# facebookresearch/EgoT2

Measured on AMD Instinct MI355X. Metric: clips/sec fwd+bwd, 3-task TTM translator (B=256,T=15,d=128), higher is better.
Workload: dtype f32 (operands split exactly into 3 bf16 parts; 6 bf16 MFMA products per K-block, f32 accumulate); 1 GPU; configs[1]: TTM 3-task translator, 1 layer d=128 h=4 d_ff=2048, B=256/GPU T=15 S=45, synthetic N(0,1) features, random-init weights, train mode dropout=0.5 (+0.1 on PE), weighted CE (evaluated in the forward's head epilogue), fwd+bwd; global_batch=256, parallelism=dp1, impl=auto, workgroups_per_clip=1, launch=one hipGraph replay per step, deterministic=False, compute_is_module_default=True, loss=weighted CE in the forward's head epilogue (egx_ce)

## Files before the change

### egot2_amd/csrc/fused_bwd.hip

```cpp
#include <stdlib.h>
#include <string.h>
#include <type_traits>
#include "common.h"
#include "kernels.h"
#include "fused.h"
#ifndef EGX_FFN_PIPE_BWD
#define EGX_FFN_PIPE_BWD 0
#endif
#ifndef EGX_FFN_PIPE_BWD_RING
#define EGX_FFN_PIPE_BWD_RING 16
#endif

#ifdef EGX_STAMPS
namespace egx { extern __device__ unsigned long long g_bstamps[32]; }
#define LNB_STAMP(base, k) do { if ((base) >= 0 && blockIdx.x == 0 && threadIdx.x == 0) { __builtin_amdgcn_sched_barrier(0); egx::g_bstamps[(base) + (k)] = __builtin_amdgcn_s_memtime(); __builtin_amdgcn_sched_barrier(0); } } while (0)
#endif
#include "fused_dev.h"

namespace egx {

template <int CM, int HT>
__global__ __launch_bounds__(256, HT == 1 ? 2 : 1) void ffn_dw_kernel(FfnDwParams p) {
    extern __shared__ __attribute__((aligned(16))) float lds[];
    constexpr int TILE = 32 * LDX;
// ... 1195 lines not shown
        const float* tile0 = p.slabs + (size_t)(pr.first_block + item * pr.splits) * (64 * 128) + r * 128 + c;
        float4 s = make_float4(0, 0, 0, 0);
        int sp = 0;
        for (; sp + 8 <= nsp; sp += 8) {
            float4 v[8];
#pragma unroll
            for (int k = 0; k < 8; ++k) v[k] = *reinterpret_cast<const float4*>(tile0 + (size_t)(sp + k) * (64 * 128));
#pragma unroll
            for (int k = 0; k < 8; ++k) { s.x += v[k].x; s.y += v[k].y; s.z += v[k].z; s.w += v[k].w; }
        }
        for (; sp < nsp; ++sp) {
            const float4 v = *reinterpret_cast<const float4*>(tile0 + (size_t)sp * (64 * 128));
            s.x += v.x; s.y += v.y; s.z += v.z; s.w += v.w;
        }
        const int row = row0 + r, col = col0 + c;
        if (row < pr.R && col < pr.C) {
            float4* dst = reinterpret_cast<float4*>(pr.out + (size_t)row * pr.C + col);
            const float4 o = *dst;
            *dst = make_float4(o.x + s.x, o.y + s.y, o.z + s.z, o.w + s.w);
        }
        return;
    }
    reduce_slabs_block(t.red, b - t.part_blocks - t.tile_blocks);
}

int tail_reduce(const SmallDwParams* sp, const SlabReduce* red, const ReducePartialsParams* rp, uint64_t* seed_advance_ptr, const TouchList* touch, hipStream_t st) {
    TailReduceParams t;
    memset(&t, 0, sizeof(t));
    if (sp && sp->n && sp->slabs) {
        t.sp = *sp;
        int items = 0;
        for (int i = 0; i < sp->n; ++i) items += cdiv(sp->pr[i].R, 64) * cdiv(sp->pr[i].C, 128);
        t.tile_blocks = (unsigned)items * 8;
    }
    if (red && red->narr) {
        t.red = *red;
        size_t total = 0;
        for (int k = 0; k < red->narr; ++k) total += red->n[k];
        t.slab_blocks = (unsigned)((total / 4 + 255) / 256);
    }
    if (rp && rp->n) { t.rp = *rp; t.part_blocks = (unsigned)cdiv(rp->P, 16); }
    t.seed_advance = seed_advance_ptr;
    if (touch) t.touch = *touch;
    const unsigned blocks = t.tile_blocks + t.slab_blocks + t.part_blocks;
    if (!blocks) return seed_advance_ptr ? seed_advance(seed_advance_ptr, st) : 0;
    hipLaunchKernelGGL(tail_reduce_kernel, dim3(blocks), dim3(256), 0, st, t);
    EGX_LAUNCH_CHECK();
    return 0;
}

__device__ unsigned g_stolen_bwd;
long long slices_stolen_bwd(int reset) {
    unsigned v = 0;
    if (hipMemcpyFromSymbol(&v, HIP_SYMBOL(g_stolen_bwd), sizeof(v)) != hipSuccess) return -1;
    if (reset) { const unsigned z = 0; (void)hipMemcpyToSymbol(HIP_SYMBOL(g_stolen_bwd), &z, sizeof(z)); }
    return v;
}
__device__ unsigned long long g_bstamps[32];
#ifdef EGX_STAMPS
#define BSTAMP(i) do { if (blockIdx.x == 0 && threadIdx.x == 0) g_bstamps[i] = __builtin_amdgcn_s_memtime(); } while (0)
#else
#define BSTAMP(i) do { } while (0)
#endif
int debug_read_bstamps(unsigned long long* out, int n) {
    return hipMemcpyFromSymbol(out, HIP_SYMBOL(g_bstamps), sizeof(unsigned long long) * (n > 32 ? 32 : n)) == hipSuccess ? 0 : 1;
}

template <int CM, bool TILED, int DH, bool SLICED = false, bool CUT = false, bool RAGGED = false>
__global__ __launch_bounds__(256, 1) void fused_bwd_kernel(FusedBwdParams p) {
    static_assert(!(TILED && SLICED), "the tiled launches are not sliced");
    static_assert(!RAGGED || TILED, "ragged batches run the tiled launches");
    static_assert(!(CUT && (TILED || SLICED)), "the cut launches are neither tiled nor sliced");
    constexpr int HPW = FDH / DH, NHEAD = FH * HPW, NCT = DH / 16;
    constexpr int NT = 3;
    constexpr int SP = NT * 16;
    constexpr int BLK = SP * LDX;
    extern __shared__ __attribute__((aligned(16))) float lds[];
    float* Gs = lds;
    float* B1 = lds + 1 * BLK;
    float* B2 = lds + 2 * BLK;
    float* B3 = lds + 3 * BLK;
    float* B4 = lds + 4 * BLK;
    float* B5 = lds + 5 * BLK;
    float* stat = lds + 6 * BLK;
    float* PSB = stat + NHEAD * 3 * SP;

    const int tid = threadIdx.x, wave = tid >> 6;
    int lane = tid & 63, r = lane & 15, q = lane >> 4;
    int clip_ = blockIdx.x, slice_ = 0;
    if constexpr (SLICED) slice_map(p.n_slices, clip_, slice_);
    const int clip = clip_, slice = slice_;
    const int n_slices = SLICED ? p.n_slices : 1;
    int S, c_real, t0;
    size_t tok0;
    const int* rrec = nullptr;
    if constexpr (RAGGED) {
        c_real = p.rtab[(size_t)p.B_clips * RAGGED_REC + clip];
        rrec = p.rtab + (size_t)c_real * RAGGED_REC;
        t0 = (clip - rrec[RG_TILE0]) * 48;
        S = min(48, rrec[RG_S] - t0);
        tok0 = (size_t)rrec[RG_TOK0] + t0;
    } else if constexpr (TILED) {
        c_real = clip / p.tpc;
        t0 = (clip - c_real * p.tpc) * 48;
        S = min(48, p.S_clip - t0);
        tok0 = (size_t)c_real * p.S_clip + t0;
    } else {
        c_real = clip; t0 = 0; S = p.S; tok0 = (size_t)clip * S;
    }
    if (!CUT && p.zero_buf) {
        const size_t n4 = p.zero_n / 4, per = (n4 + gridDim.x - 1) / gridDim.x;
        const size_t b0 = (size_t)blockIdx.x * per, b1 = b0 + per < n4 ? b0 + per : n4;
        for (size_t k = b0 + threadIdx.x; k < b1; k += 256) reinterpret_cast<float4*>(p.zero_buf)[k] = make_float4(0, 0, 0, 0);
    }
    if constexpr (SLICED) { if (clip >= p.B || ((p.slice_drop >> slice) & 1)) return; }

    BSTAMP(12);
    float* part = p.partials + (size_t)clip * p.P;
#define EGX_PHASE()                                              \
    do {                                                         \
        int t_ = threadIdx.x;                                    \
        asm volatile("" : "+v"(t_));                             \
        lane = t_ & 63; r = lane & 15; q = lane >> 4;            \
    } while (0)

    const bool dev_seed = p.seed_ptr != nullptr;
    const uint64_t seed_dev = dev_seed ? *p.seed_ptr : 0ull;
    const uint64_t pos_key = dev_seed ? site_key(seed_dev, 0, SITE_POS) : p.pos_key;
    constexpr int BPF = SP * (FD / 4) / 256;
    static_assert(SP * (FD / 4) % 256 == 0, "a block must divide among the threads");
    auto blk_request = [&](f32x4 (&v)[BPF], const float* src) {
        int t_ = threadIdx.x;
        asm volatile("" : "+v"(t_));
        const f32x4* s4 = reinterpret_cast<const f32x4*>(src);
        const int n = S * (FD / 4);
#pragma unroll
        for (int k = 0; k < BPF; ++k) { const int i = t_ + 256 * k; v[k] = s4[i < n ? i : n - 1]; }
    };
    auto blk_store = [&](const f32x4 (&v)[BPF], float* dst, float* dst2) {
        int t_ = threadIdx.x;
        asm volatile("" : "+v"(t_));
#pragma unroll
        for (int k = 0; k < BPF; ++k) {
            const int i = t_ + 256 * k, row = i >> 5, c = (i & 31) << 2;
            if (i < S * (FD / 4)) {
                *reinterpret_cast<f32x4*>(dst + row * LDX + c) = v[k];
                if (dst2) *reinterpret_cast<f32x4*>(dst2 + row * LDX + c) = v[k];
            }
        }
    };
    f32x4 pf_a[BPF], pf_b[BPF];
    auto res_ptr = [&](int slot) -> const float* {
        return TILED ? p.saved_res + ((size_t)slot * p.Ntok + tok0) * FD : p.saved_res + ((size_t)slot * p.B + clip) * S * FD;
    };
    const int l_first = CUT ? p.cut_layer : TILED ? p.l_back : p.n_layers - 1;
    Touched tch = {{0, 0, 0, 0}};
    if constexpr (!TILED) { if (p.touch.n) tch = touch_lines<256>(p.touch, blockIdx.x, gridDim.x, tid); }
    blk_request(pf_a, CUT ? p.dy1 + tok0 * FD : l_first >= 0 ? res_ptr(2 * l_first + 1) : p.saved_pre + tok0 * FD);
    blk_request(pf_b, l_first >= 0 ? res_ptr(2 * l_first) : p.saved_pre + tok0 * FD);
    const int ps_g = tid >> 5, ps_c = (tid & 31) << 2;
    const f32x4 ln0_v = *reinterpret_cast<const f32x4*>(p.ln_w + ps_c);
    f32x4 n1_v = *reinterpret_cast<const f32x4*>(p.layer[l_first >= 0 ? l_first : 0].norm1_w + ps_c);
    static_assert((6 * BLK) % 4 == 0, "the blocks are zeroed in 16-byte pieces");
    for (int i = tid; i < 6 * BLK / 4; i += 256) reinterpret_cast<f32x4*>(lds)[i] = f32x4{0, 0, 0, 0};
    if (ps_g == 0) *reinterpret_cast<f32x4*>(PSB + ps_c) = ln0_v;
    __syncthreads();
    if constexpr (TILED) {
        if (p.l_front >= 0) {
// ... 617 lines not shown
                for (int j = 0; j < 32; ++j) dy[j] += t[j];
                load32(B4 + row * LDX + c0, t);
#pragma unroll
                for (int j = 0; j < 32; ++j) dy[j] += t[j];
                load32(B1 + row * LDX + c0, t);
#pragma unroll
                for (int j = 0; j < 32; ++j) dy[j] += t[j];
                load32(B5 + row * LDX + c0, x);
            },
            [&](int row, int c0, float (&dy)[32], float (&dx)[32], float (&dyx)[32]) {
                store32(Gs + row * LDX + c0, dy);
                store32(B1 + row * LDX + c0, dx);
                store32(B4 + row * LDX + c0, dyx);
                if (w.res_thresh) {
                    uint32_t orow = (uint32_t)(tok0 + row);
#pragma unroll
                    for (int j = 0; j < 32; ++j) dx[j] *= drop_scale(k_res1, orow, (uint32_t)(c0 + j), w.res_thresh, w.drop_inv);
                }
                store32(B2 + row * LDX + c0, dx);
            },
            [&] {
                if constexpr (!TILED) {
                    int t_ = threadIdx.x;
                    asm volatile("" : "+v"(t_));
#pragma unroll
                    for (int k = 0; k < QKV_PF; ++k) qv[k] = qsrc[t_ + 256 * k];
                }
            }, 16);
        BSTAMP(21);
        __syncthreads();
        store_block(w.g1_out + tok0 * FD, B2, S);
        BSTAMP(5);
        PackW<CM, 2, 4> wo_pf;
        pack_issue(wo_pf, w.out_proj_wtp, wave * 2, 4, 0);
        if (tid < 128) {
            pl[384 + tid] = colsum_lds(B4, 0, S, tid);
            pl[640 + tid] = colsum_lds(B2, 0, S, tid);
        } else {
            pl[512 + (tid - 128)] = colsum_lds(Gs, 0, S, tid - 128);
        }
        EGX_PHASE();
        __syncthreads();
        {
            f32x4 acc[2][NT];
#pragma unroll
            for (int i = 0; i < 2; ++i)
#pragma unroll
                for (int t = 0; t < NT; ++t) acc[i][t] = f32x4{0, 0, 0, 0};
            gemm_packed<CM, 2, NT, 4>(acc, wo_pf, B2, r, q);
#pragma unroll
            for (int i = 0; i < 2; ++i)
#pragma unroll
                for (int t = 0; t < NT; ++t)
                    *reinterpret_cast<float4*>(B3 + (t * 16 + r) * LDX + (wave * 2 + i) * 16 + 4 * q) =
                        make_float4(acc[i][t][0], acc[i][t][1], acc[i][t][2], acc[i][t][3]);
        }
        BSTAMP(6);
        if constexpr (TILED) {
            __syncthreads();
            store_block(p.datt + tok0 * FD, B3, S);
            store_block(p.dres + tok0 * FD, B1, S);
            return;
        }
        {
            int t_ = threadIdx.x;
            asm volatile("" : "+v"(t_));
#pragma unroll
            for (int k = 0; k < QKV_PF; ++k) {
                const int i = t_ + 256 * k, row = i / 96, c = (i - row * 96) * 4;
                float* dst = c < FD ? B4 + c : (c < 2 * FD ? B5 + (c - FD) : Gs + (c - 2 * FD));
                *reinterpret_cast<f32x4*>(dst + row * LDX) = qv[k];
            }
        }
        __syncthreads();
        BSTAMP(7);
        EGX_PHASE();
        BSTAMP(8);
        EGX_PHASE();
#pragma unroll
        for (int hl = 0; hl < HPW; ++hl) {
            const int h = wave * HPW + hl;
            const int hc = h * DH;
            const float scale = DH == 32 ? 0.17677669529663687f : 0.25f;
            float* st_m = stat + (h * 3 + 0) * SP;
            float* st_i = stat + (h * 3 + 1) * SP;
            float* st_d = stat + (h * 3 + 2) * SP;
            Frag<CM> fq[NT], fk[NT], fv[NT], fdo[NT];
#pragma unroll
            for (int t = 0; t < NT; ++t) {
                fq[t] = load_head_frag<CM, DH>(B4 + (t * 16 + r) * LDX + hc, q);
                fk[t] = load_head_frag<CM, DH>(B5 + (t * 16 + r) * LDX + hc, q);
                fv[t] = load_head_frag<CM, DH>(Gs + (t * 16 + r) * LDX + hc, q);
                fdo[t] = load_head_frag<CM, DH>(B3 + (t * 16 + r) * LDX + hc, q);
            }
            auto ldq = [&](int t) -> const Frag<CM>& { return fq[t]; };
            auto ldk = [&](int t) -> const Frag<CM>& { return fk[t]; };
            auto ldv = [&](int t) -> const Frag<CM>& { return fv[t]; };
            auto ldo = [&](int t) -> const Frag<CM>& { return fdo[t]; };
            f32x4 pt[NT][NT], dpt[NT][NT];
#pragma unroll
            for (int qt = 0; qt < NT; ++qt) {
                Frag<CM> bq = ldq(qt), bdo = ldo(qt);
#pragma unroll
                for (int kt = 0; kt < NT; ++kt) {
                    pt[kt][qt] = f32x4{0, 0, 0, 0};
                    dpt[kt][qt] = f32x4{0, 0, 0, 0};
                    mma<CM>(pt[kt][qt], ldk(kt), bq);
                    mma<CM>(dpt[kt][qt], ldv(kt), bdo);
                }
            }
            auto keep = [&](int query, int key) -> float {
                return w.attn_thresh ? drop_scale(k_attn, (uint32_t)((clip * NHEAD + h) * 64 + query), (uint32_t)key, w.attn_thresh, w.drop_inv) : 1.f;
            };
#pragma unroll
            for (int qt = 0; qt < NT; ++qt) {
                float m = -INFINITY;
#pragma unroll
                for (int kt = 0; kt < NT; ++kt)
#pragma unroll
                    for (int e = 0; e < 4; ++e) {
                        int key = kt * 16 + 4 * q + e;
                        float sv = (key < S) ? pt[kt][qt][e] * scale : -INFINITY;
                        pt[kt][qt][e] = sv;
                        m = fmaxf(m, sv);
                    }
                m = fmaxf(m, __shfl_xor(m, 16, 64));
                m = fmaxf(m, __shfl_xor(m, 32, 64));
                float sum = 0.f;
#pragma unroll
                for (int kt = 0; kt < NT; ++kt)
#pragma unroll
                    for (int e = 0; e < 4; ++e) { float pv = __expf(pt[kt][qt][e] - m); pt[kt][qt][e] = pv; sum += pv; }
                sum += __shfl_xor(sum, 16, 64);
                sum += __shfl_xor(sum, 32, 64);
                float inv = 1.f / sum;
                int query = qt * 16 + r;
                float dl = 0.f;
                float ksv[NT][4];
#pragma unroll
                for (int kt = 0; kt < NT; ++kt)
#pragma unroll
                    for (int e = 0; e < 4; ++e) {
                        float pv = pt[kt][qt][e] * inv;
                        float ks = keep(query, kt * 16 + 4 * q + e);
                        ksv[kt][e] = ks;
                        pt[kt][qt][e] = pv;
                        dpt[kt][qt][e] *= ks;
                        dl += pv * dpt[kt][qt][e];
                    }
                dl += __shfl_xor(dl, 16, 64);
                dl += __shfl_xor(dl, 32, 64);
                if (q == 0) { st_m[query] = m; st_i[query] = inv; st_d[query] = dl; }
#pragma unroll
                for (int kt = 0; kt < NT; ++kt)
#pragma unroll
                    for (int e = 0; e < 4; ++e) {
                        float pv = pt[kt][qt][e];
                        dpt[kt][qt][e] = pv * (dpt[kt][qt][e] - dl) * scale;
                        pt[kt][qt][e] = pv * ksv[kt][e];
                    }
            }
            f32x4 oq[NCT][NT], dqa[NCT][NT];
#pragma unroll
            for (int ct = 0; ct < NCT; ++ct)
#pragma unroll
                for (int qt = 0; qt < NT; ++qt) { oq[ct][qt] = f32x4{0, 0, 0, 0}; dqa[ct][qt] = f32x4{0, 0, 0, 0}; }
#pragma unroll
            for (int kb = 0; kb < 2; ++kb) {
                Frag<CM> av[NCT], ak[NCT];
#pragma unroll
                for (int ct = 0; ct < NCT; ++ct) {
                    av[ct] = gather_frag<CM>(Gs, hc + ct * 16 + r, kb * 32, q, SP - 1);
                    ak[ct] = gather_frag<CM>(B5, hc + ct * 16 + r, kb * 32, q, SP - 1);
                }
#pragma unroll
                for (int qt = 0; qt < NT; ++qt) {
                    f32x4 z = f32x4{0, 0, 0, 0};
                    Frag<CM> bp = chain_frag<CM>(pt[2 * kb][qt], (2 * kb + 1 < NT) ? pt[(2 * kb + 1 < NT) ? 2 * kb + 1 : 0][qt] : z);
                    Frag<CM> bs = chain_frag<CM>(dpt[2 * kb][qt], (2 * kb + 1 < NT) ? dpt[(2 * kb + 1 < NT) ? 2 * kb + 1 : 0][qt] : z);
#pragma unroll
                    for (int ct = 0; ct < NCT; ++ct) {
                        mma<CM>(oq[ct][qt], av[ct], bp);
                        mma<CM>(dqa[ct][qt], ak[ct], bs);
                    }
                }
            }
#pragma unroll
            for (int ct = 0; ct < NCT; ++ct)
#pragma unroll
                for (int qt = 0; qt < NT; ++qt) {
                    int tok = qt * 16 + r;
                    if (tok < S)
                        *reinterpret_cast<float4*>(w.attn_o_out + (tok0 + tok) * FD + hc + ct * 16 + 4 * q) =
                            make_float4(oq[ct][qt][0], oq[ct][qt][1], oq[ct][qt][2], oq[ct][qt][3]);
                }
            f32x4 pn[NT][NT], dsn[NT][NT];
#pragma unroll
            for (int qt = 0; qt < NT; ++qt) {
                float4 m4 = *reinterpret_cast<const float4*>(st_m + qt * 16 + 4 * q);
                float4 i4 = *reinterpret_cast<const float4*>(st_i + qt * 16 + 4 * q);
                float4 d4 = *reinterpret_cast<const float4*>(st_d + qt * 16 + 4 * q);
                float mq[4] = {m4.x, m4.y, m4.z, m4.w}, iq[4] = {i4.x, i4.y, i4.z, i4.w}, dq4[4] = {d4.x, d4.y, d4.z, d4.w};
#pragma unroll
                for (int kt = 0; kt < NT; ++kt) {
                    f32x4 sN = f32x4{0, 0, 0, 0}, dN = f32x4{0, 0, 0, 0};
                    mma<CM>(sN, ldq(qt), ldk(kt));
                    mma<CM>(dN, ldo(qt), ldv(kt));
                    int key = kt * 16 + r;
                    uint32_t m4[4] = {0xFu, 0xFu, 0xFu, 0xFu};
                    if (w.attn_thresh) tile_keep_rows(k_attn, (uint32_t)((clip * NHEAD + h) * 64 + qt * 16), (uint32_t)(kt * 4), r, q, w.attn_thresh, m4);
                    const float kinv = w.attn_thresh ? w.drop_inv : 1.f;
#pragma unroll
                    for (int e = 0; e < 4; ++e) {
                        int query = qt * 16 + 4 * q + e;
                        bool ok = (key < S) && (query < S);
                        float pv = ok ? __expf(sN[e] * scale - mq[e]) * iq[e] : 0.f;
                        float ks = ((m4[e] >> (r & 3)) & 1u) ? kinv : 0.f;
                        pn[qt][kt][e] = pv * ks;
                        dsn[qt][kt][e] = pv * (ks * dN[e] - dq4[e]) * scale;
                    }
                }
            }
            f32x4 dva[NCT][NT], dka[NCT][NT];
#pragma unroll
            for (int ct = 0; ct < NCT; ++ct)
#pragma unroll
                for (int kt = 0; kt < NT; ++kt) { dva[ct][kt] = f32x4{0, 0, 0, 0}; dka[ct][kt] = f32x4{0, 0, 0, 0}; }
#pragma unroll
            for (int kb = 0; kb < 2; ++kb) {
                Frag<CM> ad[NCT], aq[NCT];
#pragma unroll
                for (int ct = 0; ct < NCT; ++ct) {
                    ad[ct] = gather_frag<CM>(B3, hc + ct * 16 + r, kb * 32, q, SP - 1);
                    aq[ct] = gather_frag<CM>(B4, hc + ct * 16 + r, kb * 32, q, SP - 1);
                }
#pragma unroll
                for (int kt = 0; kt < NT; ++kt) {
                    f32x4 z = f32x4{0, 0, 0, 0};
                    Frag<CM> bp = chain_frag<CM>(pn[2 * kb][kt], (2 * kb + 1 < NT) ? pn[(2 * kb + 1 < NT) ? 2 * kb + 1 : 0][kt] : z);
                    Frag<CM> bs = chain_frag<CM>(dsn[2 * kb][kt], (2 * kb + 1 < NT) ? dsn[(2 * kb + 1 < NT) ? 2 * kb + 1 : 0][kt] : z);
#pragma unroll
                    for (int ct = 0; ct < NCT; ++ct) {
                        mma<CM>(dva[ct][kt], ad[ct], bp);
                        mma<CM>(dka[ct][kt], aq[ct], bs);
                    }
                }
            }
#pragma unroll
            for (int ct = 0; ct < NCT; ++ct)
#pragma unroll
                for (int t = 0; t < NT; ++t) {
                    int tok = t * 16 + r;
                    int c = hc + ct * 16 + 4 * q;
                    bool tv = tok < S;
                    float4 vq = tv ? make_float4(dqa[ct][t][0], dqa[ct][t][1], dqa[ct][t][2], dqa[ct][t][3]) : make_float4(0, 0, 0, 0);
                    float4 vk = tv ? make_float4(dka[ct][t][0], dka[ct][t][1], dka[ct][t][2], dka[ct][t][3]) : make_float4(0, 0, 0, 0);
                    float4 vv = tv ? make_float4(dva[ct][t][0], dva[ct][t][1], dva[ct][t][2], dva[ct][t][3]) : make_float4(0, 0, 0, 0);
                    *reinterpret_cast<float4*>(B4 + tok * LDX + c) = vq;
                    *reinterpret_cast<float4*>(B5 + tok * LDX + c) = vk;
                    *reinterpret_cast<float4*>(Gs + tok * LDX + c) = vv;
                    if (tv) {
                        float* o = w.dqkv_out + (tok0 + tok) * (3 * FD) + c;
                        *reinterpret_cast<float4*>(o) = vq;
                        *reinterpret_cast<float4*>(o + FD) = vk;
                        *reinterpret_cast<float4*>(o + 2 * FD) = vv;
                    }
                }
        }
        __syncthreads();
        BSTAMP(9);
        PackW<CM, 2, 4> wi_pf;
        pack_issue(wi_pf, w.in_proj_wtp, wave * 2, 12, 0);
        blk_request(pf_a, l > 0 ? res_ptr(2 * (l - 1) + 1) : p.saved_pre + tok0 * FD);
        blk_request(pf_b, l > 0 ? res_ptr(2 * (l - 1)) : p.saved_pre + tok0 * FD);
        if (tid < 128) {
            pl[768 + tid] = colsum_lds(B4, 0, S, tid);
            pl[768 + 256 + tid] = colsum_lds(Gs, 0, S, tid);
        } else {
            pl[768 + 128 + (tid - 128)] = colsum_lds(B5, 0, S, tid - 128);
        }
        EGX_PHASE();
        {
            f32x4 acc[2][NT];
#pragma unroll
            for (int i = 0; i < 2; ++i)
#pragma unroll
                for (int t = 0; t < NT; ++t) acc[i][t] = f32x4{0, 0, 0, 0};
            PackW<CM, 2, 4> wi2, wi3;
            pack_issue(wi2, w.in_proj_wtp, wave * 2, 12, 4);
            gemm_packed<CM, 2, NT, 4>(acc, wi_pf, B4, r, q);
            pack_issue(wi3, w.in_proj_wtp, wave * 2, 12, 8);
            gemm_packed<CM, 2, NT, 4>(acc, wi2, B5, r, q);
            gemm_packed<CM, 2, NT, 4>(acc, wi3, Gs, r, q);
#pragma unroll
            for (int i = 0; i < 2; ++i)
#pragma unroll
                for (int t = 0; t < NT; ++t) {
                    int tok = t * 16 + r;
                    int c = (wave * 2 + i) * 16 + 4 * q;
                    float4 rs = *reinterpret_cast<const float4*>(B1 + tok * LDX + c);
                    float4 o = make_float4(acc[i][t][0] + rs.x, acc[i][t][1] + rs.y, acc[i][t][2] + rs.z, acc[i][t][3] + rs.w);
                    if (tok >= S) o = make_float4(0, 0, 0, 0);
                    *reinterpret_cast<float4*>(B2 + tok * LDX + c) = o;
                }
        }
        __syncthreads();
        { float* t = Gs; Gs = B2; B2 = t; }
        if constexpr (CUT) {
            if (l > 0) {
                store_block(p.dxin + tok0 * FD, Gs, S);
                return;
            }
        }
    }

        BSTAMP(10);
    {
        float* pg = part + p.n_layers * FUSED_P_LAYER;
        blk_store(pf_a, B1, nullptr);
        __syncthreads();
        ln_bwd_rows_lds(S, PSB, p.eps,
            [&](int row, int c0, float (&dy)[32], float (&x)[32]) {
                load32(Gs + row * LDX + c0, dy);
                if (p.pos_thresh) {
                    uint32_t orow = (uint32_t)(tok0 + row);
#pragma unroll
                    for (int j = 0; j < 32; ++j) dy[j] *= drop_scale(pos_key, orow, (uint32_t)(c0 + j), p.pos_thresh, p.pos_inv);
                }
                load32(B1 + row * LDX + c0, x);
            },
            [&](int row, int c0, float (&dy)[32], float (&dx)[32], float (&dyx)[32]) {
                store32(Gs + row * LDX + c0, dy);
                store32(B3 + row * LDX + c0, dyx);
                if (!RAGGED && p.feat_thresh) {
#pragma unroll
                    for (int si = 0; si < FUSED_MAX_SEG; ++si)
                        if (si < p.nseg && t0 + row >= p.seg[si].off && t0 + row < p.seg[si].off + p.seg[si].T) {
                            const size_t frow = (size_t)c_real * p.seg[si].T + (t0 + row - p.seg[si].off);
                            const uint64_t fk = dev_seed ? site_key(seed_dev, (uint32_t)si, SITE_FEAT) : p.feat_key[si];
#pragma unroll
                            for (int j = 0; j < 32; ++j) dx[j] *= drop_scale(fk, (uint32_t)frow, (uint32_t)(c0 + j), p.feat_thresh, p.feat_inv);
                        }
                }
                store32(B1 + row * LDX + c0, dx);
            }, [] {}, 22);
        BSTAMP(27);
        __syncthreads();
#pragma unroll
        for (int si = 0; si < FUSED_MAX_SEG; ++si)
            if (si < p.nseg) {
                const int soff = RAGGED ? rrec[RG_OFF + si] : p.seg[si].off, sT = RAGGED ? rrec[RG_T + si] : p.seg[si].T;
                int r0 = soff - t0, r1 = r0 + sT;
                const int lo = max(r0, 0), hi = min(r1, S);
                float* dst = p.dseg_out[si] + ((RAGGED ? (size_t)p.rseg[(size_t)c_real * FUSED_MAX_SEG + si] : (size_t)c_real * sT) + (lo - r0)) * FD;
                for (int i = tid; i < (hi - lo) * (FD / 4); i += 256) {
                    const int row = lo + (i >> 5), c4 = i & 31;
                    *reinterpret_cast<float4*>(dst + (size_t)i * 4) = *reinterpret_cast<const float4*>(B1 + row * LDX + c4 * 4);
                }
            }
        if (p.dx0_out) store_block(p.dx0_out + tok0 * FD, Gs, S);
        if (tid < 128) pg[tid] = colsum_lds(B3, 0, S, tid);
        else pg[128 + (tid - 128)] = colsum_lds(Gs, 0, S, tid - 128);
        for (int si = 0; si < p.nseg; ++si) {
            int r0 = (RAGGED ? rrec[RG_OFF + si] : p.seg[si].off) - t0, r1 = r0 + (RAGGED ? rrec[RG_T + si] : p.seg[si].T);
            r0 = max(r0, 0); r1 = min(r1, S);
            if (tid < 128) pg[256 + si * 256 + tid] = colsum_lds(Gs, r0, r1, tid);
            else pg[256 + si * 256 + 128 + (tid - 128)] = colsum_lds(B1, r0, r1, tid - 128);
        }
    }
    BSTAMP(11);
}

__global__ __launch_bounds__(256) void reduce_partials_kernel(ReducePartialsParams rp) {
    reduce_partials_block(rp, blockIdx.x, blockIdx.y, gridDim.y);
}

int reduce_partials(const ReducePartialsParams& rp, hipStream_t st, bool deterministic) {
    hipLaunchKernelGGL(reduce_partials_kernel, dim3(cdiv(rp.P, 64), deterministic ? 1 : partial_chunks(rp.B)), dim3(256), 0, st, rp);
    EGX_LAUNCH_CHECK();
    return 0;
}

template <int CM, bool TILED, int DH>
static int launch_bwd(const FusedBwdParams& p, hipStream_t st) {
    size_t lds = (size_t)(6 * 48 * LDX + (FH * FDH / DH) * 3 * 48 + 2 * FD) * sizeof(float);
    static bool attr_set = false;
    if (!attr_set) {
        EGX_HIP(hipFuncSetAttribute(reinterpret_cast<const void*>(&fused_bwd_kernel<CM, TILED, DH>),
                                    hipFuncAttributeMaxDynamicSharedMemorySize, (int)lds));
        if constexpr (!TILED)
            EGX_HIP(hipFuncSetAttribute(reinterpret_cast<const void*>(&fused_bwd_kernel<CM, false, DH, true>),
                                        hipFuncAttributeMaxDynamicSharedMemorySize, (int)lds));
        attr_set = true;
    }
    timing_begin(TIMER_FUSED_BWD, st);
    bool sliced = false;
    if constexpr (!TILED) sliced = p.n_slices > 1;
    if constexpr (!TILED) {
        if (p.cut) {
            static bool cut_attr = false;
            if (!cut_attr) {
                EGX_HIP(hipFuncSetAttribute(reinterpret_cast<const void*>(&fused_bwd_kernel<CM, false, DH, false, true>),
                                            hipFuncAttributeMaxDynamicSharedMemorySize, (int)lds));
                cut_attr = true;
            }
            EGX_CHECK(!sliced && p.dy1 && (p.cut_layer == 0 || p.dxin), "cut mode: one workgroup per clip, dy1 / dxin set");
            hipLaunchKernelGGL((fused_bwd_kernel<CM, false, DH, false, true>), dim3(p.B), dim3(256), lds, st, p);
            timing_end(TIMER_FUSED_BWD, st);
            EGX_LAUNCH_CHECK();
            return 0;
        }
    }
    if (sliced) {
        if constexpr (!TILED)
            hipLaunchKernelGGL((fused_bwd_kernel<CM, false, DH, true>), dim3((p.B + 7) / 8 * 8 * p.n_slices), dim3(256), lds, st, p);
    } else {
        hipLaunchKernelGGL((fused_bwd_kernel<CM, TILED, DH>), dim3(p.B), dim3(256), lds, st, p);
    }
    timing_end(TIMER_FUSED_BWD, st);
    EGX_LAUNCH_CHECK();
    return 0;
}

template <int CM>
static int launch_bwd_ragged(const FusedBwdParams& p, hipStream_t st) {
    EGX_CHECK(p.S == 48 && p.rtab && p.rseg, "fused backward: ragged launch needs S = 48 and the batch table");
    const size_t lds = (size_t)(6 * 48 * LDX + FH * 3 * 48 + 2 * FD) * sizeof(float);
    static bool attr_set = false;
    if (!attr_set) {
        EGX_HIP(hipFuncSetAttribute(reinterpret_cast<const void*>(&fused_bwd_kernel<CM, true, 32, false, false, true>),
                                    hipFuncAttributeMaxDynamicSharedMemorySize, (int)lds));
        attr_set = true;
    }
    timing_begin(TIMER_FUSED_BWD, st);
    hipLaunchKernelGGL((fused_bwd_kernel<CM, true, 32, false, false, true>), dim3(p.B), dim3(256), lds, st, p);
    timing_end(TIMER_FUSED_BWD, st);
    EGX_LAUNCH_CHECK();
    return 0;
}

int fused_backward(const FusedBwdParams& p, int compute, hipStream_t st) {
    EGX_CHECK(p.S <= 48, "fused backward: S=%d > 48", p.S);
    if (p.tiled) {
        EGX_CHECK(compute == CM_BF16 || compute == CM_SPLIT, "tiled mode: compute must be bf16 or f32s");
        if (p.rtab) return compute == CM_BF16 ? launch_bwd_ragged<CM_BF16>(p, st) : launch_bwd_ragged<CM_SPLIT>(p, st);
        return compute == CM_BF16 ? launch_bwd<CM_BF16, true, 32>(p, st) : launch_bwd<CM_SPLIT, true, 32>(p, st);
    }
    if (p.n_heads == 2 * FH)
        return compute == CM_BF16 ? launch_bwd<CM_BF16, false, 16>(p, st) : compute == CM_SPLIT ? launch_bwd<CM_SPLIT, false, 16>(p, st) : launch_bwd<CM_F32, false, 16>(p, st);
    return compute == CM_BF16 ? launch_bwd<CM_BF16, false, 32>(p, st) : compute == CM_SPLIT ? launch_bwd<CM_SPLIT, false, 32>(p, st) : launch_bwd<CM_F32, false, 32>(p, st);
}

}
```

### egot2_amd/csrc/fused_dev.h

```cpp
#pragma once
#include "common.h"
#include "fused.h"

namespace egx {

constexpr int FD = 128;
constexpr int FH = 4;
constexpr int FDH = 32;
constexpr int LDX = FD + 4;
constexpr int LDV = 64 + 4;

enum { CM_F32 = 0, CM_BF16 = 1, CM_SPLIT = 2 };
typedef uint32_t u32x4 __attribute__((ext_vector_type(4)));

template <int CM> struct Frag { float v[8]; };
template <> struct Frag<CM_BF16> { bf16x8 v; };
template <> struct Frag<CM_SPLIT> { bf16x8 p[3]; };

__device__ __forceinline__ uint32_t pack_bf16(float a, float b) { return pack_bf16x2(a, b); }

__device__ __forceinline__ void split_pair(float x, float y, uint32_t& h, uint32_t& m, uint32_t& l) {
    typedef float f32x2 __attribute__((ext_vector_type(2)));
    h = pack_bf16(x, y);
    f32x2 v = {x, y};
// ... 104 lines not shown
__device__ __forceinline__ void pin(WRaw<CM_SPLIT>& x) {
#pragma unroll
    for (int i = 0; i < 3; ++i) asm volatile("" : "+v"(x.p[i]));
}
template <class T, int N>
__device__ __forceinline__ void pin_all(T (&x)[N]) {
#pragma unroll
    for (int i = 0; i < N; ++i) pin(x[i]);
}
template <class T, int N, int M>
__device__ __forceinline__ void pin_all(T (&x)[N][M]) {
#pragma unroll
    for (int i = 0; i < N; ++i)
#pragma unroll
        for (int j = 0; j < M; ++j) pin(x[i][j]);
}


constexpr int LDXH = FD + 4;
__device__ __forceinline__ void split32(const float (&v)[32], uint32_t (&h)[16], uint32_t (&m)[16], uint32_t (&l)[16]) {
#pragma unroll
    for (int j = 0; j < 16; ++j) split_pair(v[2 * j], v[2 * j + 1], h[j], m[j], l[j]);
}
__device__ __forceinline__ void store_parts32(unsigned short* d, size_t plane_stride, const uint32_t (&h)[16], const uint32_t (&m)[16],
                                              const uint32_t (&l)[16]) {
#pragma unroll
    for (int g = 0; g < 8; ++g) {
        *reinterpret_cast<uint2*>(d + 4 * g) = make_uint2(h[2 * g], h[2 * g + 1]);
        *reinterpret_cast<uint2*>(d + plane_stride + 4 * g) = make_uint2(m[2 * g], m[2 * g + 1]);
        *reinterpret_cast<uint2*>(d + 2 * plane_stride + 4 * g) = make_uint2(l[2 * g], l[2 * g + 1]);
    }
}
__device__ __forceinline__ void store_split32(unsigned short* planes, int plane_stride, int row, int c0, const float (&v)[32]) {
    uint32_t h[16], m[16], l[16];
    split32(v, h, m, l);
    store_parts32(planes + row * LDXH + c0, (size_t)plane_stride, h, m, l);
}
__device__ __forceinline__ Frag<CM_SPLIT> load_split_frag(const unsigned short* planes, int plane_stride, int row, int k0, int q) {
    Frag<CM_SPLIT> f;
#pragma unroll
    for (int i = 0; i < 3; ++i) {
        const unsigned short* b = planes + i * plane_stride + row * LDXH + k0 + 4 * q;
        uint2 lo = *reinterpret_cast<const uint2*>(b);
        uint2 hi = *reinterpret_cast<const uint2*>(b + 16);
        f.p[i] = __builtin_bit_cast(bf16x8, (u32x4){lo.x, lo.y, hi.x, hi.y});
    }
    return f;
}

template <int CM>
__device__ __forceinline__ Frag<CM> chain_frag(const f32x4& t0, const f32x4& t1) {
    return make_frag<CM>(make_float4(t0[0], t0[1], t0[2], t0[3]), make_float4(t1[0], t1[1], t1[2], t1[3]));
}

template <int CM>
__device__ __forceinline__ void mma(f32x4& acc, const Frag<CM>& a, const Frag<CM>& b) {
    if constexpr (CM == CM_BF16) {
        acc = __builtin_amdgcn_mfma_f32_16x16x32_bf16(a.v, b.v, acc, 0, 0, 0);
    } else if constexpr (CM == CM_SPLIT) {
        acc = __builtin_amdgcn_mfma_f32_16x16x32_bf16(a.p[2], b.p[0], acc, 0, 0, 0);
        acc = __builtin_amdgcn_mfma_f32_16x16x32_bf16(a.p[1], b.p[1], acc, 0, 0, 0);
        acc = __builtin_amdgcn_mfma_f32_16x16x32_bf16(a.p[0], b.p[2], acc, 0, 0, 0);
        acc = __builtin_amdgcn_mfma_f32_16x16x32_bf16(a.p[1], b.p[0], acc, 0, 0, 0);
        acc = __builtin_amdgcn_mfma_f32_16x16x32_bf16(a.p[0], b.p[1], acc, 0, 0, 0);
        acc = __builtin_amdgcn_mfma_f32_16x16x32_bf16(a.p[0], b.p[0], acc, 0, 0, 0);
    } else {
#pragma unroll
        for (int j = 0; j < 8; ++j) acc = __builtin_amdgcn_mfma_f32_16x16x4f32(a.v[j], b.v[j], acc, 0, 0, 0);
    }
}

template <int CTRL>
__device__ __forceinline__ float dpp_quad(float v) {
    return __builtin_bit_cast(float, __builtin_amdgcn_mov_dpp(__builtin_bit_cast(int, v), CTRL, 0xF, 0xF, true));
}
__device__ __forceinline__ void quad_transpose(float (&v)[4], int lane) {
    const bool h2 = (lane & 2) != 0, h1 = (lane & 1) != 0;
    const float t0 = dpp_quad<0x4E>(v[0]), t1 = dpp_quad<0x4E>(v[1]);
    const float t2 = dpp_quad<0x4E>(v[2]), t3 = dpp_quad<0x4E>(v[3]);
    const float w0 = h2 ? t2 : v[0], w1 = h2 ? t3 : v[1], w2 = h2 ? v[2] : t0, w3 = h2 ? v[3] : t1;
    const float u0 = dpp_quad<0xB1>(w0), u1 = dpp_quad<0xB1>(w1);
    const float u2 = dpp_quad<0xB1>(w2), u3 = dpp_quad<0xB1>(w3);
    v[0] = h1 ? u1 : w0; v[1] = h1 ? w1 : u0; v[2] = h1 ? u3 : w2; v[3] = h1 ? w3 : u2;
}
constexpr int HTILE_ELEMS = 256;
template <int CM>
__device__ __forceinline__ void store_hid_tile(void* tile, const f32x4& c, int lane, int n_valid) {
    float v[4] = {c[0], c[1], c[2], c[3]};
    if constexpr (CM == CM_BF16) {
        if (__builtin_amdgcn_readfirstlane(n_valid) < 16) {
            asm volatile("" ::: "memory");
            const bool ok = (lane & 15) < n_valid;
#pragma unroll
            for (int j = 0; j < 4; ++j) v[j] = ok ? v[j] : 0.f;
        }
        reinterpret_cast<uint2*>(tile)[lane] = make_uint2(pack_bf16(v[0], v[1]), pack_bf16(v[2], v[3]));
        return;
    }
    quad_transpose(v, lane);
    const int r = lane & 15, q = lane >> 4;
    const int t0 = 4 * (r >> 2);
    if (__builtin_amdgcn_readfirstlane(n_valid) < 16) {
        asm volatile("" ::: "memory");
#pragma unroll
        for (int j = 0; j < 4; ++j) v[j] = (t0 + j < n_valid) ? v[j] : 0.f;
    }
    const int dst = 4 * q + (r & 3) + 16 * (r >> 2);
    if constexpr (CM == CM_BF16) {
        reinterpret_cast<uint2*>(tile)[dst] = make_uint2(pack_bf16(v[0], v[1]), pack_bf16(v[2], v[3]));
    } else {
        reinterpret_cast<float4*>(tile)[dst] = make_float4(v[0], v[1], v[2], v[3]);
    }
}
__device__ __forceinline__ void store_hid_tile_bf16(void* tile0, u32x4 u, int lane, int n_valid) {
    if (__builtin_amdgcn_readfirstlane(n_valid) < 16) {
        asm volatile("" ::: "memory");
        const bool ok = (lane & 15) < n_valid;
#pragma unroll
        for (int j = 0; j < 4; ++j) u[j] = ok ? u[j] : 0u;
    }
    reinterpret_cast<uint2*>(tile0)[lane] = make_uint2(u[0], u[1]);
    reinterpret_cast<uint2*>(tile0)[64 + lane] = make_uint2(u[2], u[3]);
}
template <int CM>
__device__ __forceinline__ Frag<CM> load_hid_frag(const void* tile_a, const void* tile_b, int lane) {
    if constexpr (CM == CM_BF16) {
        Frag<CM> f;
        uint2 a = reinterpret_cast<const uint2*>(tile_a)[lane];
        uint2 b = reinterpret_cast<const uint2*>(tile_b)[lane];
        u32x4 u = {a.x, a.y, b.x, b.y};
        f.v = __builtin_bit_cast(bf16x8, u);
        return f;
    } else {
        float4 a = reinterpret_cast<const float4*>(tile_a)[lane];
        float4 b = reinterpret_cast<const float4*>(tile_b)[lane];
        return make_frag<CM>(a, b);
    }
}

__device__ __forceinline__ float wsum(float v) {
#pragma unroll
    for (int o = 32; o > 0; o >>= 1) v += __shfl_xor(v, o, 64);
    return v;
}

struct Touched { uint32_t v[TOUCH_MAX]; };
template <int NTHREADS>
__device__ __forceinline__ Touched touch_lines(const TouchList& tl, int block, int nblocks, int tid) {
    Touched t;
#pragma unroll
    for (int k = 0; k < TOUCH_MAX; ++k) {
        const int kk = k < tl.n ? k : 0;
        const unsigned nl = tl.lines[kk], per = (nl + (unsigned)nblocks - 1) / (unsigned)nblocks;
        unsigned i = (unsigned)block * per + (unsigned)tid;
        i = (i < nl && (unsigned)tid < per) ? i : nl - 1;
        t.v[k] = *reinterpret_cast<const uint32_t*>(reinterpret_cast<const char*>(tl.base[kk]) + ((size_t)i << 7));
    }
    return t;
}
__device__ __forceinline__ void touch_sink(const Touched& t) {
#pragma unroll
    for (int k = 0; k < TOUCH_MAX; ++k) asm volatile("" :: "v"(t.v[k]));
}

__device__ __forceinline__ float wmax(float v) {
#pragma unroll
// ... 434 lines not shown
```

Baseline: 708,000 clips/s.

## Transpose attention P/dS tiles in registers instead of recomputing transposed scores

The attention backward used to compute the transposed probability and dS tiles a second time: it redid the QK^T and dO·V^T MFMAs, re-evaluated exp and the dropout mask, and read per-query softmax stats back from LDS. It now takes the already-computed P and dS tiles and transposes them in registers with a DPP quad transpose followed by ds_bpermute. This removes the LDS stats buffer and the Q/dO fragment arrays that had to stay live, easing register and LDS pressure. In exchange each tile pays extra cross-lane permutes, and padded query rows are now zeroed explicitly.

Result: no change. 711,700 clips/s, median of 6 (+0.5%).

```diff
diff --git a/egot2_amd/csrc/fused_bwd.hip b/egot2_amd/csrc/fused_bwd.hip
--- a/egot2_amd/csrc/fused_bwd.hip
+++ b/egot2_amd/csrc/fused_bwd.hip
@@ -1301,8 +1301,7 @@
     float* B3 = lds + 3 * BLK;
     float* B4 = lds + 4 * BLK;
     float* B5 = lds + 5 * BLK;
-    float* stat = lds + 6 * BLK;
-    float* PSB = stat + NHEAD * 3 * SP;
+    float* PSB = lds + 6 * BLK;
 
     const int tid = threadIdx.x, wave = tid >> 6;
     int lane = tid & 63, r = lane & 15, q = lane >> 4;
@@ -2086,31 +2085,23 @@
             const int h = wave * HPW + hl;
             const int hc = h * DH;
             const float scale = DH == 32 ? 0.17677669529663687f : 0.25f;
-            float* st_m = stat + (h * 3 + 0) * SP;
-            float* st_i = stat + (h * 3 + 1) * SP;
-            float* st_d = stat + (h * 3 + 2) * SP;
-            Frag<CM> fq[NT], fk[NT], fv[NT], fdo[NT];
+            Frag<CM> fk[NT], fv[NT];
 #pragma unroll
             for (int t = 0; t < NT; ++t) {
-                fq[t] = load_head_frag<CM, DH>(B4 + (t * 16 + r) * LDX + hc, q);
                 fk[t] = load_head_frag<CM, DH>(B5 + (t * 16 + r) * LDX + hc, q);
                 fv[t] = load_head_frag<CM, DH>(Gs + (t * 16 + r) * LDX + hc, q);
-                fdo[t] = load_head_frag<CM, DH>(B3 + (t * 16 + r) * LDX + hc, q);
-            }
-            auto ldq = [&](int t) -> const Frag<CM>& { return fq[t]; };
-            auto ldk = [&](int t) -> const Frag<CM>& { return fk[t]; };
-            auto ldv = [&](int t) -> const Frag<CM>& { return fv[t]; };
-            auto ldo = [&](int t) -> const Frag<CM>& { return fdo[t]; };
+            }
             f32x4 pt[NT][NT], dpt[NT][NT];
 #pragma unroll
             for (int qt = 0; qt < NT; ++qt) {
-                Frag<CM> bq = ldq(qt), bdo = ldo(qt);
+                const Frag<CM> bq = load_head_frag<CM, DH>(B4 + (qt * 16 + r) * LDX + hc, q);
+                const Frag<CM> bdo = load_head_frag<CM, DH>(B3 + (qt * 16 + r) * LDX + hc, q);
 #pragma unroll
                 for (int kt = 0; kt < NT; ++kt) {
                     pt[kt][qt] = f32x4{0, 0, 0, 0};
                     dpt[kt][qt] = f32x4{0, 0, 0, 0};
-                    mma<CM>(pt[kt][qt], ldk(kt), bq);
-                    mma<CM>(dpt[kt][qt], ldv(kt), bdo);
+                    mma<CM>(pt[kt][qt], fk[kt], bq);
+                    mma<CM>(dpt[kt][qt], fv[kt], bdo);
                 }
             }
             auto keep = [&](int query, int key) -> float {
@@ -2154,14 +2145,14 @@
                     }
                 dl += __shfl_xor(dl, 16, 64);
                 dl += __shfl_xor(dl, 32, 64);
-                if (q == 0) { st_m[query] = m; st_i[query] = inv; st_d[query] = dl; }
+                const bool qok = query < S;
 #pragma unroll
                 for (int kt = 0; kt < NT; ++kt)
 #pragma unroll
                     for (int e = 0; e < 4; ++e) {
                         float pv = pt[kt][qt][e];
-                        dpt[kt][qt][e] = pv * (dpt[kt][qt][e] - dl) * scale;
-                        pt[kt][qt][e] = pv * ksv[kt][e];
+                        dpt[kt][qt][e] = qok ? pv * (dpt[kt][qt][e] - dl) * scale : 0.f;
+                        pt[kt][qt][e] = qok ? pv * ksv[kt][e] : 0.f;
                     }
             }
             f32x4 oq[NCT][NT], dqa[NCT][NT];
@@ -2200,31 +2191,14 @@
                 }
             f32x4 pn[NT][NT], dsn[NT][NT];
 #pragma unroll
-            for (int qt = 0; qt < NT; ++qt) {
-                float4 m4 = *reinterpret_cast<const float4*>(st_m + qt * 16 + 4 * q);
-                float4 i4 = *reinterpret_cast<const float4*>(st_i + qt * 16 + 4 * q);
-                float4 d4 = *reinterpret_cast<const float4*>(st_d + qt * 16 + 4 * q);
-                float mq[4] = {m4.x, m4.y, m4.z, m4.w}, iq[4] = {i4.x, i4.y, i4.z, i4.w}, dq4[4] = {d4.x, d4.y, d4.z, d4.w};
+            for (int qt = 0; qt < NT; ++qt)
 #pragma unroll
                 for (int kt = 0; kt < NT; ++kt) {
-                    f32x4 sN = f32x4{0, 0, 0, 0}, dN = f32x4{0, 0, 0, 0};
-                    mma<CM>(sN, ldq(qt), ldk(kt));
-                    mma<CM>(dN, ldo(qt), ldv(kt));
-                    int key = kt * 16 + r;
-                    uint32_t m4[4] = {0xFu, 0xFu, 0xFu, 0xFu};
-                    if (w.attn_thresh) tile_keep_rows(k_attn, (uint32_t)((clip * NHEAD + h) * 64 + qt * 16), (uint32_t)(kt * 4), r, q, w.attn_thresh, m4);
-                    const float kinv = w.attn_thresh ? w.drop_inv : 1.f;
-#pragma unroll
-                    for (int e = 0; e < 4; ++e) {
-                        int query = qt * 16 + 4 * q + e;
-                        bool ok = (key < S) && (query < S);
-                        float pv = ok ? __expf(sN[e] * scale - mq[e]) * iq[e] : 0.f;
-                        float ks = ((m4[e] >> (r & 3)) & 1u) ? kinv : 0.f;
-                        pn[qt][kt][e] = pv * ks;
-                        dsn[qt][kt][e] = pv * (ks * dN[e] - dq4[e]) * scale;
-                    }
-                }
-            }
+                    pn[qt][kt] = pt[kt][qt];
+                    dsn[qt][kt] = dpt[kt][qt];
+                    tile_transpose(pn[qt][kt], lane);
+                    tile_transpose(dsn[qt][kt], lane);
+                }
             f32x4 dva[NCT][NT], dka[NCT][NT];
 #pragma unroll
             for (int ct = 0; ct < NCT; ++ct)
@@ -2387,7 +2361,7 @@
 
 template <int CM, bool TILED, int DH>
 static int launch_bwd(const FusedBwdParams& p, hipStream_t st) {
-    size_t lds = (size_t)(6 * 48 * LDX + (FH * FDH / DH) * 3 * 48 + 2 * FD) * sizeof(float);
+    size_t lds = (size_t)(6 * 48 * LDX + 2 * FD) * sizeof(float);
     static bool attr_set = false;
     if (!attr_set) {
         EGX_HIP(hipFuncSetAttribute(reinterpret_cast<const void*>(&fused_bwd_kernel<CM, TILED, DH>),
@@ -2429,7 +2403,7 @@
 template <int CM>
 static int launch_bwd_ragged(const FusedBwdParams& p, hipStream_t st) {
     EGX_CHECK(p.S == 48 && p.rtab && p.rseg, "fused backward: ragged launch needs S = 48 and the batch table");
-    const size_t lds = (size_t)(6 * 48 * LDX + FH * 3 * 48 + 2 * FD) * sizeof(float);
+    const size_t lds = (size_t)(6 * 48 * LDX + 2 * FD) * sizeof(float);
     static bool attr_set = false;
     if (!attr_set) {
         EGX_HIP(hipFuncSetAttribute(reinterpret_cast<const void*>(&fused_bwd_kernel<CM, true, 32, false, false, true>),
diff --git a/egot2_amd/csrc/fused_dev.h b/egot2_amd/csrc/fused_dev.h
--- a/egot2_amd/csrc/fused_dev.h
+++ b/egot2_amd/csrc/fused_dev.h
@@ -210,6 +210,13 @@
     const float u0 = dpp_quad<0xB1>(w0), u1 = dpp_quad<0xB1>(w1);
     const float u2 = dpp_quad<0xB1>(w2), u3 = dpp_quad<0xB1>(w3);
     v[0] = h1 ? u1 : w0; v[1] = h1 ? w1 : u0; v[2] = h1 ? u3 : w2; v[3] = h1 ? w3 : u2;
+}
+__device__ __forceinline__ void tile_transpose(f32x4& t, int lane) {
+    float v[4] = {t[0], t[1], t[2], t[3]};
+    quad_transpose(v, lane);
+    const int src = ((((lane >> 2) & 3) << 4) | ((lane >> 4) << 2) | (lane & 3)) << 2;
+#pragma unroll
+    for (int e = 0; e < 4; ++e) t[e] = __int_as_float(__builtin_amdgcn_ds_bpermute(src, __float_as_int(v[e])));
 }
 constexpr int HTILE_ELEMS = 256;
 template <int CM>
```

## Reuse packed P/dS fragments via LDS transpose instead of recomputing attention for dK/dV

Applied to the files above, without the earlier changes.

For the bf16 and split-bf16 paths, the attention backward no longer recomputes the transposed score and dP tiles (two extra MFMA passes plus exp and dropout masks) to form the dV and dK operands. It stages the already packed P and dS fragments into per-wave LDS and reads them back transposed with ds_read_tr16_b64. Dropout masks are now generated four at a time with drop_scale4, and padded query rows are zeroed explicitly. The trade is extra LDS traffic and wave-local syncs, plus more live fragment registers, in exchange for skipping the recompute.

Result: faster. 710,700 clips/s before, 718,200 clips/s after (median of 6 runs) (+1.0%).

```diff
diff --git a/egot2_amd/csrc/fused_bwd.hip b/egot2_amd/csrc/fused_bwd.hip
--- a/egot2_amd/csrc/fused_bwd.hip
+++ b/egot2_amd/csrc/fused_bwd.hip
@@ -2113,9 +2113,6 @@
                     mma<CM>(dpt[kt][qt], ldv(kt), bdo);
                 }
             }
-            auto keep = [&](int query, int key) -> float {
-                return w.attn_thresh ? drop_scale(k_attn, (uint32_t)((clip * NHEAD + h) * 64 + query), (uint32_t)key, w.attn_thresh, w.drop_inv) : 1.f;
-            };
 #pragma unroll
             for (int qt = 0; qt < NT; ++qt) {
                 float m = -INFINITY;
@@ -2142,19 +2139,22 @@
                 float dl = 0.f;
                 float ksv[NT][4];
 #pragma unroll
+                for (int kt = 0; kt < NT; ++kt) {
+                    if (w.attn_thresh) drop_scale4(k_attn, (uint32_t)((clip * NHEAD + h) * 64 + query), (uint32_t)(kt * 16 + 4 * q), w.attn_thresh, w.drop_inv, ksv[kt]);
+                    else ksv[kt][0] = ksv[kt][1] = ksv[kt][2] = ksv[kt][3] = 1.f;
+                }
+#pragma unroll
                 for (int kt = 0; kt < NT; ++kt)
 #pragma unroll
                     for (int e = 0; e < 4; ++e) {
                         float pv = pt[kt][qt][e] * inv;
-                        float ks = keep(query, kt * 16 + 4 * q + e);
-                        ksv[kt][e] = ks;
                         pt[kt][qt][e] = pv;
-                        dpt[kt][qt][e] *= ks;
+                        dpt[kt][qt][e] *= ksv[kt][e];
                         dl += pv * dpt[kt][qt][e];
                     }
                 dl += __shfl_xor(dl, 16, 64);
                 dl += __shfl_xor(dl, 32, 64);
-                if (q == 0) { st_m[query] = m; st_i[query] = inv; st_d[query] = dl; }
+                if constexpr (CM == CM_F32) { if (q == 0) { st_m[query] = m; st_i[query] = inv; st_d[query] = dl; } }
 #pragma unroll
                 for (int kt = 0; kt < NT; ++kt)
 #pragma unroll
@@ -2163,8 +2163,18 @@
                         dpt[kt][qt][e] = pv * (dpt[kt][qt][e] - dl) * scale;
                         pt[kt][qt][e] = pv * ksv[kt][e];
                     }
+                if ((qt + 1) * 16 > S) {
+#pragma unroll
+                    for (int kt = 0; kt < NT; ++kt)
+#pragma unroll
+                        for (int e = 0; e < 4; ++e) {
+                            pt[kt][qt][e] = query < S ? pt[kt][qt][e] : 0.f;
+                            dpt[kt][qt][e] = query < S ? dpt[kt][qt][e] : 0.f;
+                        }
+                }
             }
             f32x4 oq[NCT][NT], dqa[NCT][NT];
+            Frag<CM> cp[2][NT], cs[2][NT];
 #pragma unroll
             for (int ct = 0; ct < NCT; ++ct)
 #pragma unroll
@@ -2180,12 +2190,12 @@
 #pragma unroll
                 for (int qt = 0; qt < NT; ++qt) {
                     f32x4 z = f32x4{0, 0, 0, 0};
-                    Frag<CM> bp = chain_frag<CM>(pt[2 * kb][qt], (2 * kb + 1 < NT) ? pt[(2 * kb + 1 < NT) ? 2 * kb + 1 : 0][qt] : z);
-                    Frag<CM> bs = chain_frag<CM>(dpt[2 * kb][qt], (2 * kb + 1 < NT) ? dpt[(2 * kb + 1 < NT) ? 2 * kb + 1 : 0][qt] : z);
+                    cp[kb][qt] = chain_frag<CM>(pt[2 * kb][qt], (2 * kb + 1 < NT) ? pt[(2 * kb + 1 < NT) ? 2 * kb + 1 : 0][qt] : z);
+                    cs[kb][qt] = chain_frag<CM>(dpt[2 * kb][qt], (2 * kb + 1 < NT) ? dpt[(2 * kb + 1 < NT) ? 2 * kb + 1 : 0][qt] : z);
 #pragma unroll
                     for (int ct = 0; ct < NCT; ++ct) {
-                        mma<CM>(oq[ct][qt], av[ct], bp);
-                        mma<CM>(dqa[ct][qt], ak[ct], bs);
+                        mma<CM>(oq[ct][qt], av[ct], cp[kb][qt]);
+                        mma<CM>(dqa[ct][qt], ak[ct], cs[kb][qt]);
                     }
                 }
             }
@@ -2198,6 +2208,63 @@
                         *reinterpret_cast<float4*>(w.attn_o_out + (tok0 + tok) * FD + hc + ct * 16 + 4 * q) =
                             make_float4(oq[ct][qt][0], oq[ct][qt][1], oq[ct][qt][2], oq[ct][qt][3]);
                 }
+            f32x4 dva[NCT][NT], dka[NCT][NT];
+#pragma unroll
+            for (int ct = 0; ct < NCT; ++ct)
+#pragma unroll
+                for (int kt = 0; kt < NT; ++kt) { dva[ct][kt] = f32x4{0, 0, 0, 0}; dka[ct][kt] = f32x4{0, 0, 0, 0}; }
+            if constexpr (CM != CM_F32) {
+            constexpr int NPL = CM == CM_SPLIT ? 3 : 1, TRP = SP * 16;
+            static_assert(4 * NPL * TRP * 2 <= BLK * 4, "the per-wave P / dS tiles must fit in one LDS block");
+            typedef short s4v __attribute__((ext_vector_type(4)));
+            typedef __attribute__((address_space(3))) s4v lds_s4v;
+            unsigned short* tb = reinterpret_cast<unsigned short*>(B2) + wave * (NPL * TRP);
+            auto tr_off = [](int row, int chunk) { return row * 16 + 4 * (chunk ^ ((row >> 2) & 3)); };
+            Frag<CM> ad[2][NCT], aq[2][NCT];
+#pragma unroll
+            for (int kb = 0; kb < 2; ++kb)
+#pragma unroll
+                for (int ct = 0; ct < NCT; ++ct) {
+                    ad[kb][ct] = gather_frag<CM>(B3, hc + ct * 16 + r, kb * 32, q, SP - 1);
+                    aq[kb][ct] = gather_frag<CM>(B4, hc + ct * 16 + r, kb * 32, q, SP - 1);
+                }
+            auto wave_lds_sync = [] {
+                __builtin_amdgcn_wave_barrier();
+                asm volatile("s_waitcnt lgkmcnt(0)" ::: "memory");
+            };
+            auto stage_tile = [&](const Frag<CM> (&c)[2][NT], const Frag<CM> (&a)[2][NCT], f32x4 (&acc)[NCT][NT], int kt) {
+#pragma unroll
+                for (int qt = 0; qt < NT; ++qt)
+#pragma unroll
+                    for (int pl = 0; pl < NPL; ++pl) {
+                        u32x4 u;
+                        if constexpr (CM == CM_SPLIT) u = __builtin_bit_cast(u32x4, c[kt >> 1][qt].p[pl]);
+                        else u = __builtin_bit_cast(u32x4, c[kt >> 1][qt].v);
+                        *reinterpret_cast<uint2*>(tb + pl * TRP + tr_off(qt * 16 + r, q)) = (kt & 1) ? make_uint2(u[2], u[3]) : make_uint2(u[0], u[1]);
+                    }
+                wave_lds_sync();
+#pragma unroll
+                for (int kb = 0; kb < 2; ++kb) {
+                    Frag<CM> b;
+                    const unsigned short* s = tb + tr_off(kb * 32 + 4 * q + (r >> 2), r & 3);
+#pragma unroll
+                    for (int pl = 0; pl < NPL; ++pl) {
+                        const s4v lo = __builtin_amdgcn_ds_read_tr16_b64_v4i16((lds_s4v*)(s + pl * TRP));
+                        const s4v hi = kb == 0 ? __builtin_amdgcn_ds_read_tr16_b64_v4i16((lds_s4v*)(s + pl * TRP + 16 * 16)) : s4v{0, 0, 0, 0};
+                        const bf16x8 v = __builtin_bit_cast(bf16x8, __builtin_shufflevector(lo, hi, 0, 1, 2, 3, 4, 5, 6, 7));
+                        if constexpr (CM == CM_SPLIT) b.p[pl] = v; else b.v = v;
+                    }
+#pragma unroll
+                    for (int ct = 0; ct < NCT; ++ct) mma<CM>(acc[ct][kt], a[kb][ct], b);
+                }
+                wave_lds_sync();
+            };
+#pragma unroll
+            for (int kt = 0; kt < NT; ++kt) {
+                stage_tile(cp, ad, dva, kt);
+                stage_tile(cs, aq, dka, kt);
+            }
+            } else {
             f32x4 pn[NT][NT], dsn[NT][NT];
 #pragma unroll
             for (int qt = 0; qt < NT; ++qt) {
@@ -2225,11 +2292,6 @@
                     }
                 }
             }
-            f32x4 dva[NCT][NT], dka[NCT][NT];
-#pragma unroll
-            for (int ct = 0; ct < NCT; ++ct)
-#pragma unroll
-                for (int kt = 0; kt < NT; ++kt) { dva[ct][kt] = f32x4{0, 0, 0, 0}; dka[ct][kt] = f32x4{0, 0, 0, 0}; }
 #pragma unroll
             for (int kb = 0; kb < 2; ++kb) {
                 Frag<CM> ad[NCT], aq[NCT];
@@ -2249,6 +2311,7 @@
                         mma<CM>(dka[ct][kt], aq[ct], bs);
                     }
                 }
+            }
             }
 #pragma unroll
             for (int ct = 0; ct < NCT; ++ct)
```
